# wangtong627/COR

Measured on AMD Instinct MI355X. Metric: query triplets/sec (forward + similarity + top-k), higher is better.
Workload: dtype bf16

## Files before the change

cor_amd/_native.py:

```python
from __future__ import annotations

import ctypes as C
import os

_HERE = os.path.dirname(os.path.abspath(__file__))
LIB_PATH = os.environ.get("COR_AMD_LIB") or os.path.join(_HERE, "csrc", "libcor_amd.so")

F32, BF16, F16, BF16X3 = 0, 1, 2, 3
ACT_NONE, ACT_GELU_ERF, ACT_RELU, ACT_SIGMOID, ACT_GELU_TANH = 0, 1, 2, 3, 4
EINVAL, ENOSUPPORT = -1, -2
TOPK_FORCE_LISTS, TOPK_NO_FALLBACK, TOPK_FORCE_GLOBAL_THRESHOLD, TOPK_WAVE_FINAL = 1, 2, 8, 16
TOPK_KMAX = 256
FILTER_EQ, FILTER_NE = 0, 1
MERGE_NMAX = 4096
EXPAND_SEGMAX = 16
ORDER_REVERSE = 1 << 30
KERNEL_ROWLANE, KERNEL_FEWQ, KERNEL_FLASH_MFMA, KERNEL_FLASH_PIPELINED, KERNEL_WINDOW_BLOCK = 1, 2, 3, 4, 5
import numpy as _np
Q_PRESCALE_HD64 = float(_np.float32(0.125) * _np.float32(1.4426950408889634))

_p, _i, _l, _f, _ll = C.c_void_p, C.c_int, C.c_long, C.c_float, C.c_longlong

SIGNATURES = {
    "cor_version": [],
    "cor_gemm": [_p, _l, _p, _l, _i, _p, _l, _i, _i, _i, _i, _p, _i, _p, _p, _l, _i, _i, _p],
    "cor_layernorm": [_p, _i, _p, _i, _p, _p, _i, _i, _f, _i, _p],
    "cor_attention": [_p, _l, _l, _p, _l, _l, _p, _l, _l, _i, _p, _l, _l, _i, _i, _i, _i, _i, _i, _f, _p],
    "cor_attention_f32": [_p, _l, _l, _p, _l, _l, _p, _l, _l, _p, _l, _l, _i, _i, _i, _i, _i, _i, _f, _p],
    "cor_attention_kernel_id": [_i, _i, _i, _i, _i, _i],
    "cor_sam_attention": [_p, _i, _p, _i, _p, _p, _p, _i, _i, _i, _i, _i, _f, _i, _p],
    "cor_patchify": [_p, _p, _i, _i, _i, _i, _i, _i, _i, _p],
    "cor_im2col3x3": [_p, _i, _p, _i, _i, _i, _i, _p],
    "cor_add": [_p, _i, _p, _i, _p, _i, _l, _l, _p],
    "cor_copy_rows": [_p, _l, _i, _p, _l, _i, _i, _i, _p],
    "cor_split_x3": [_p, _l, _p, _l, _l, _i, _i, _p],
    "cor_tokens_to_nchw": [_p, _i, _p, _i, _i, _i, _p],
    "cor_nchw_to_tokens": [_p, _p, _i, _i, _i, _i, _p],
    "cor_l2norm_rows": [_p, _i, _p, _i, _i, _i, _f, _p],
    "cor_embed_tokens": [_p, _p, _p, _p, _i, _i, _i, _i, _p],
    "cor_bilinear": [_p, _p, _i, _i, _i, _i, _i, _i, _p],
    "cor_conv3x3s2_small": [_p, _i, _p, _p, _p, _i, _i, _i, _i, _i, _p],
    "cor_dwconv7x7": [_p, _p, _p, _p, _i, _i, _i, _i, _i, _p],
    "cor_adapter_pool": [_p, _p, _p, _i, _i, _i, _i, _p],
    "cor_masked_pool": [_p, _i, _p, _p, _i, _i, _i, _i, _i, _p],
    "cor_region_pool": [_p, _p, _p, _p, _i, _i, _i, _i, _i, _i, _i, _p],
    "cor_fuse_gate": [_p, _p, _p, _p, _p, _i, _i, _p],
    "cor_fuse_mix": [_p, _p, _p, _i, _i, _p],
    "cor_dense_pe": [_p, _p, _i, _i, _p],
    "cor_upscale_shuffle": [_p, _i, _p, _p, _p, _f, _i, _p, _i, _i, _i, _i, _i, _p],
    "cor_upscale_hyper": [_p, _i, _p, _p, _p, _l, _p, _i, _i, _i, _i, _i, _i, _p],
    "cor_iou_select": [_p, _p, _i, _i, _i, _i, _i, _p, _p, _p],
    "cor_decoder_heads": [_p, _p, _p, _p, _p, _i, _p, _p, _i, _p],
    "cor_mask_prob_minmax": [_p, _p, _i, _i, _p],
    "cor_resize_binarize": [_p, _p, _i, _i, _i, _i, _i, _f, _p],
    "cor_resize_gray": [_p, _p, _i, _i, _i, _i, _i, _p],
# ... 60 lines not shown
```

cor_amd/csrc/flash_attn.hip:

```cpp
#include <cstdlib>
#include <type_traits>

#include "common.h"

typedef short s16x4 __attribute__((ext_vector_type(4)));

namespace {

struct FlashArgs {
  const bf16_t* q; const bf16_t* k; const bf16_t* v; void* o;
  long q_sb, q_st, k_sb, k_st, v_sb, v_st, o_sb, o_st;
  int H, Tq, Tk;
  float scale_log2;
  float tbl_scale;
  const bf16_t* pad_row; const float* rel_h; const float* rel_w;
  int grid, S, nW, d3;
  int nqt;
  int rev;
};

constexpr int KT = 64;
constexpr int TILE_B = KT * 128;
constexpr int KV_BYTES = 4 * TILE_B;
constexpr int AUX_PER_WAVE = 8192;
// ... 1034 lines not shown
    const unsigned lds0 = __builtin_amdgcn_readfirstlane((unsigned)(size_t)((__attribute__((address_space(3))) char*)smem));
    const int sl = lane & 7;
    long colp[2]; bool okx[2];
#pragma unroll
    for (int hf = 0; hf < 2; ++hf) {
      const int kw = min(8 * hf + (lane >> 3), 13), x = wx * 14 + kw;
      okx[hf] = x < a.grid;
      colp[hf] = ((long)b * g2 + x) * a.d3 + head * 64;
    }
#pragma unroll
    for (int i8 = 0; i8 < 8; ++i8) {
      const int i = wave * 8 + i8;
      const bool isv = i >= 28;
      const int ii = isv ? i - 28 : i, kh = ii >> 1, hf = ii & 1, y = wy * 14 + kh;
      const int chunk = isv ? (sl ^ (((lane >> 4) & 1) << 2)) : (sl ^ (4 * hf + (lane >> 4)));
      const long plane = (long)(isv ? 2 : 1) * a.H * 64 + chunk * 8;
      const bf16_t* src = (y < a.grid && okx[hf]) ? a.q + colp[hf] + (long)y * a.grid * a.d3 + plane : a.pad_row + head * 64 + plane;
      glds16(src, lds0 + (isv ? WIN_KV : 0) + ii * 1024);
    }
  }

  const int tq = min(wave * 32 + r, 195);
  const int qh = (tq * 4682) >> 16, qw = tq - 14 * qh;
  uint4 qf[4];
  {
    const int y = wy * 14 + qh, x = wx * 14 + qw;
    const bf16_t* qp = (y < a.grid && x < a.grid) ? a.q + ((long)b * g2 + (long)y * a.grid + x) * a.d3 + head * 64 : a.pad_row + head * 64;
#pragma unroll
    for (int c = 0; c < 4; ++c) qf[c] = *(const uint4*)(qp + 16 * c + 8 * h);
  }

  float colb[8];
  uint4 tf[2][4];
#pragma unroll
  for (int tbl = 0; tbl < 2; ++tbl)
#pragma unroll
    for (int c = 0; c < 4; ++c) tf[tbl][c] = table_frag(tbl == 0 ? a.rel_w : a.rel_h, min(r, 26), c, h);
#pragma unroll
  for (int tbl = 0; tbl < 2; ++tbl) {
    f32x16 acc;
#pragma unroll
    for (int e = 0; e < 16; ++e) acc[e] = 0.f;
#pragma unroll
    for (int c = 0; c < 4; ++c)
      acc = __builtin_amdgcn_mfma_f32_32x32x16_bf16(__builtin_bit_cast(bf16x8, tf[tbl][c]), __builtin_bit_cast(bf16x8, qf[c]), acc, 0, 0, 0);
#pragma unroll
    for (int e = 0; e < 16; ++e) {
      const int row = acc_row(e, h);
      if (row < 27) T[row * 32 + r] = acc[e] * a.tbl_scale;
    }
    __builtin_amdgcn_fence(__ATOMIC_ACQ_REL, "wavefront");
    if (tbl == 0) {
#pragma unroll
      for (int e8 = 0; e8 < 8; ++e8) {
        const int kw = (e8 & 3) + 8 * (e8 >> 2) + 4 * h;
        colb[e8] = kw < 14 ? T[(qw - min(kw, 13) + 13) * 32 + r] : -INFINITY;
      }
      __builtin_amdgcn_fence(__ATOMIC_ACQ_REL, "wavefront");
    }
  }

  if (a.scale_log2 != 1.0f) {
#pragma unroll
    for (int c = 0; c < 4; ++c) {
      uint32_t w[4] = {qf[c].x, qf[c].y, qf[c].z, qf[c].w};
#pragma unroll
      for (int i = 0; i < 4; ++i) w[i] = pk2(__uint_as_float(w[i] << 16) * a.scale_log2, __uint_as_float(w[i] & 0xffff0000u) * a.scale_log2);
      qf[c] = make_uint4(w[0], w[1], w[2], w[3]);
    }
  }

  asm volatile("s_waitcnt vmcnt(0)" ::: "memory");
  __syncthreads();

  const int sw = (r >> 1) & 7;
  const int k_rd = r * 128, v_tr = (4 * h + ((lane & 15) >> 2)) * 128 + (16 * ((lane >> 4) & 1) + 4 * (lane & 3)) * 2;
  const int v_trd[2] = {v_tr + ((lane >> 3) & 1) * 64, v_tr + (1 - ((lane >> 3) & 1)) * 64};
  const int t_rd = (qh + 13) * 32 + r;
  f32x16 o[2], lsum;
#pragma unroll
  for (int e = 0; e < 16; ++e) { o[0][e] = 0.f; o[1][e] = 0.f; lsum[e] = 0.f; }
  float m = 0.f;
  const uint4 ones = make_uint4(0x3F803F80u, 0x3F803F80u, 0x3F803F80u, 0x3F803F80u);
#pragma unroll
  for (int blk = 0; blk < 7; ++blk) {
    const char* Kb = Kt + blk * 32 * 128 + k_rd;
    uint4 kf[4];
#pragma unroll
    for (int c = 0; c < 4; ++c) kf[c] = *(const uint4*)(Kb + (((2 * c + h) ^ sw) << 4));
    const float rm0 = T[t_rd - 32 * (2 * blk)] - m, rm1 = T[t_rd - 32 * (2 * blk + 1)] - m;
    f32x16 s;
#pragma unroll
    for (int e = 0; e < 16; ++e) s[e] = colb[e & 7] + (e < 8 ? rm0 : rm1);
#pragma unroll
    for (int c = 0; c < 4; ++c)
      s = __builtin_amdgcn_mfma_f32_32x32x16_bf16(__builtin_bit_cast(bf16x8, kf[c]), __builtin_bit_cast(bf16x8, qf[c]), s, 0, 0, 0);
// ... 234 lines not shown
```

cor_amd/csrc/gemm.hip:

```cpp
#include "common.h"

#ifdef COR_PROBES
#define COR_DBG(g_, bit_) ((g_).dbg & (bit_))
#else
#define COR_DBG(g_, bit_) 0
#endif
#ifndef COR_GEMM_DEFAULT_BIG
#define COR_GEMM_DEFAULT_BIG 2
#endif

namespace {

struct GemmArgs {
  const char* A; const char* W; char* C;
  long lda_b, ldw_b;
  long ldc;
  int M, N, Kb;
  int tm, tn;
  const float* bias; const float* col_scale; const float* residual;
  long ldr; int res_row_mod; int act;
  int group_m;
  unsigned long long* stamps;
  int dbg;
  int vec_epi;
  int rev;
  int nt_c;
  int order;
};

template <typename TA> struct Mfma;
template <> struct Mfma<float> {
  static __device__ __forceinline__ void run(const uint4& a, const uint4& b, f32x16& acc) {
    acc = __builtin_amdgcn_mfma_f32_32x32x2f32(__uint_as_float(a.x), __uint_as_float(b.x), acc, 0, 0, 0);
    acc = __builtin_amdgcn_mfma_f32_32x32x2f32(__uint_as_float(a.y), __uint_as_float(b.y), acc, 0, 0, 0);
    acc = __builtin_amdgcn_mfma_f32_32x32x2f32(__uint_as_float(a.z), __uint_as_float(b.z), acc, 0, 0, 0);
    acc = __builtin_amdgcn_mfma_f32_32x32x2f32(__uint_as_float(a.w), __uint_as_float(b.w), acc, 0, 0, 0);
  }
};
template <> struct Mfma<bf16_t> {
  static __device__ __forceinline__ void run(const uint4& a, const uint4& b, f32x16& acc) {
    acc = __builtin_amdgcn_mfma_f32_32x32x16_bf16(__builtin_bit_cast(bf16x8, a), __builtin_bit_cast(bf16x8, b), acc, 0, 0, 0);
  }
};

__device__ __forceinline__ void mfma16_bf16(const uint4& a, const uint4& b, f32x4& acc) {
  acc = __builtin_amdgcn_mfma_f32_16x16x32_bf16(__builtin_bit_cast(bf16x8, a), __builtin_bit_cast(bf16x8, b), acc, 0, 0, 0);
}

constexpr int ROWB = 128;

template <int ACT, typename TO = float> __device__ __forceinline__ float act_ct(float v) {
// ... 68 lines not shown
          st4<TO>(cp, v[0]);
        }
      }
    }
  }
}

template <typename TO, int MI, int NJ, int WTN>
__device__ __forceinline__ void epilogue_vec(const f32x16 (&acc)[MI][NJ], float* stg, const GemmArgs& g, int mbase, int nbase,
                                             int lane) {
#define COR_EPI(A_)                                                                                            \
  if (g.residual) epilogue_vec_ct<TO, MI, NJ, WTN, A_, true>(acc, stg, g, mbase, nbase, lane);                \
  else epilogue_vec_ct<TO, MI, NJ, WTN, A_, false>(acc, stg, g, mbase, nbase, lane);
  switch (g.act) {
    case COR_ACT_GELU_ERF: COR_EPI(COR_ACT_GELU_ERF) break;
    case COR_ACT_RELU: COR_EPI(COR_ACT_RELU) break;
    case COR_ACT_SIGMOID: COR_EPI(COR_ACT_SIGMOID) break;
    case COR_ACT_GELU_TANH: COR_EPI(COR_ACT_GELU_TANH) break;
    default: COR_EPI(COR_ACT_NONE) break;
  }
#undef COR_EPI
}

template <typename TA, typename TO, int BM, int BN, int WM, int WN, bool GLDS, int NBUF = 2>
__global__ void __launch_bounds__(WM * WN * 64, ((BM / WM) * (BN / WN) >= 8192 && WM * WN == 4) ? 1 : 2)
gemm_tile(const GemmArgs g) {
  constexpr int NT = WM * WN * 64;
  constexpr int WTM = BM / WM, WTN = BN / WN, MI = WTM / 32, NJ = WTN / 32;
  constexpr int A_BYTES = BM * ROWB, B_BYTES = BN * ROWB, BUF = A_BYTES + B_BYTES;
  constexpr int ACH = BM * 8 / NT, BCH = BN * 8 / NT;
  extern __shared__ __attribute__((aligned(16))) char smem[];
  const int tid = threadIdx.x, lane = tid & 63, wave = tid >> 6;
  const int wm = wave / WN, wn = wave % WN;
  const int swz0 = xcd_remap(blockIdx.x, gridDim.x);
  const int swz = g.rev ? (int)gridDim.x - 1 - swz0 : swz0;
  const int GM = g.group_m;
  const int band = swz / (GM * g.tn), rem = swz - band * (GM * g.tn);
  const int gm_eff = min(GM, g.tm - band * GM);
  const int m0 = (band * GM + rem % gm_eff) * BM, n0 = (rem / gm_eff) * BN;

  const char* a_src[ACH]; const char* b_src[BCH]; int a_ko[ACH], b_ko[BCH];
#pragma unroll
  for (int i = 0; i < ACH; ++i) {
    const int c = tid + NT * i, row = c >> 3, ch = (c & 7) ^ ((row >> 1) & 7);
    a_src[i] = g.A + (long)min(m0 + row, g.M - 1) * g.lda_b + ch * 16;
    a_ko[i] = ch * 16;
  }
#pragma unroll
  for (int i = 0; i < BCH; ++i) {
    const int c = tid + NT * i, row = c >> 3, ch = (c & 7) ^ ((row >> 1) & 7);
    b_src[i] = g.W + (long)min(n0 + row, g.N - 1) * g.ldw_b + ch * 16;
    b_ko[i] = ch * 16;
  }
  const unsigned wslot = __builtin_amdgcn_readfirstlane(tid & ~63) * 16;
  const unsigned lds0 = __builtin_amdgcn_readfirstlane((unsigned)(size_t)((__attribute__((address_space(3))) char*)smem));

  const int r = lane & 31, h = lane >> 5, sw = (lane >> 1) & 7;
  const int a_rd = (wm * WTM + r) * ROWB, b_rd = A_BYTES + (wn * WTN + r) * ROWB;
  int ch_rd[4];
#pragma unroll
  for (int s = 0; s < 4; ++s) ch_rd[s] = ((2 * s + h) ^ sw) << 4;

  f32x16 acc[MI][NJ];
#pragma unroll
  for (int i = 0; i < MI; ++i)
#pragma unroll
    for (int j = 0; j < NJ; ++j)
#pragma unroll
      for (int e = 0; e < 16; ++e) acc[i][j][e] = 0.0f;

  const int nkt = (g.Kb + ROWB - 1) / ROWB;
  uint4 ra[GLDS ? 1 : ACH], rb[GLDS ? 1 : BCH];

  auto stage_issue = [&](int kt, int buf) {
    const int kb = kt * ROWB;
    if constexpr (GLDS) {
      const unsigned base = lds0 + buf * BUF + wslot;
#pragma unroll
      for (int i = 0; i < ACH; ++i) glds16(a_src[i] + kb, base + NT * 16 * i);
#pragma unroll
      for (int i = 0; i < BCH; ++i) glds16(b_src[i] + kb, base + A_BYTES + NT * 16 * i);
    } else {
#pragma unroll
      for (int i = 0; i < ACH; ++i)
        ra[i] = (kb + a_ko[i] + 16 <= g.Kb) ? *(const uint4*)(a_src[i] + kb) : make_uint4(0, 0, 0, 0);
#pragma unroll
      for (int i = 0; i < BCH; ++i)
        rb[i] = (kb + b_ko[i] + 16 <= g.Kb) ? *(const uint4*)(b_src[i] + kb) : make_uint4(0, 0, 0, 0);
    }
  };
  auto stage_commit = [&](int buf) {
    if constexpr (!GLDS) {
      char* base = smem + buf * BUF + tid * 16;
#pragma unroll
      for (int i = 0; i < ACH; ++i) *(uint4*)(base + NT * 16 * i) = ra[i];
#pragma unroll
      for (int i = 0; i < BCH; ++i) *(uint4*)(base + A_BYTES + NT * 16 * i) = rb[i];
    }
  };
// ... 204 lines not shown
    __builtin_amdgcn_fence(__ATOMIC_ACQUIRE, "wavefront");
#pragma unroll
    for (int p4 = 0; p4 < 4; ++p4) {
      const int row = p4 * 8 + rr0;
      const uint4 q = *(const uint4*)(stg + row * 128 + ((cvr ^ ((row >> 1) & 7)) << 4));
      const int m = mbase + mi * 32 + row, n = nbase + cvr * 8;
      const unsigned off = (m < g.M && n < g.N) ? (unsigned)(((long)m * g.ldc + n) * 2L) : 0xFFFFFFFFu;
      u32x4 u; u[0] = q.x; u[1] = q.y; u[2] = q.z; u[3] = q.w;
      if constexpr (NT) __builtin_amdgcn_raw_buffer_store_b128(u, crs, off, 0, 2);
      else if (COR_DBG(g, 0x2000)) __builtin_amdgcn_raw_buffer_store_b128(u, crs, off, 0, 2);
      else if (COR_DBG(g, 0x4000)) __builtin_amdgcn_raw_buffer_store_b128(u, crs, off, 0, 16);
      else __builtin_amdgcn_raw_buffer_store_b128(u, crs, off, 0, 0);
    }
    __builtin_amdgcn_fence(__ATOMIC_RELEASE, "wavefront");
    __builtin_amdgcn_fence(__ATOMIC_ACQUIRE, "wavefront");
  }
}

#define COR_VMCNT(n_) asm volatile("s_waitcnt vmcnt(" #n_ ")" ::: "memory")

#define COR_BAR() asm volatile("s_barrier" ::: "memory")
#define COR_LGKM0() asm volatile("s_waitcnt lgkmcnt(0)" ::: "memory")

template <typename TO, bool M16>
__global__ void __launch_bounds__(512, 1) gemm_pp(const GemmArgs g) {
  constexpr int BM = 256, BN = 256, HT = 16384, NSLOT = 10;
  constexpr int MI = 4, NJ = 2, WTM = 128, WTN = 64;
  constexpr int VW = sizeof(TO) == 2 ? 8 : 4;
  constexpr int NSTORE = MI * NJ * (32 / (64 / (32 / VW)));
  static_assert(NSTORE == 16 || NSTORE == 32, "counted waits below");
  constexpr bool CT = sizeof(TO) == 2 && !M16;
  extern __shared__ __attribute__((aligned(16))) char smem[];
  const int tid = threadIdx.x, lane = tid & 63, wave = tid >> 6;
  const int wr = wave >> 2, wc = wave & 3;
  const unsigned lds0 = __builtin_amdgcn_readfirstlane((unsigned)(size_t)((__attribute__((address_space(3))) char*)smem));
  const unsigned wslot = __builtin_amdgcn_readfirstlane(wave) * 1024u;

  const int srow = tid >> 3, sch = ((tid & 7) ^ ((tid >> 4) & 7)) * 16;
  const int r = M16 ? (lane & 15) : (lane & 31), h = lane >> 5, q = lane >> 4, sw = (r >> 1) & 7;
  int chs[4];
#pragma unroll
  for (int s4 = 0; s4 < 4; ++s4) chs[s4] = M16 ? (((4 * (s4 & 1) + q) ^ sw) << 4) : (((2 * s4 + h) ^ sw) << 4);
  const int a_row = r * 128;
  const int b_row = ((wc & 1) * 64 + r) * 128;

  const int nkt = g.Kb / 128;
  const int total = g.tm * g.tn, G = gridDim.x;
  const int GM = g.group_m;
  const __amdgpu_buffer_rsrc_t crs = __builtin_amdgcn_make_buffer_rsrc(
      g.C, 0, (int)(unsigned)((((long)g.M - 1) * g.ldc + g.N) * (long)sizeof(TO)), 0x00020000);

  unsigned oa[4], ob[4];
  int m0 = 0, n0 = 0;
  const int per_xcd = (total + 7) >> 3;
// ... 180 lines not shown
      }
    };
    float* stg = (float*)(smem + 4 * HT) + wave * 1024;
    const int mb = cm0 + wr * WTM, nb = cn0 + wc * WTN;
    auto bias_col = [&](int nj, int jb) -> int { return M16 ? nj * 32 + jb * 16 + r : nj * 32 + r; };
    auto fill = [&](int mi, int nj, float* st, const float (&b)[2]) {
      if constexpr (M16) {
#pragma unroll
        for (int ib = 0; ib < 2; ++ib)
#pragma unroll
          for (int jb = 0; jb < 2; ++jb)
#pragma unroll
            for (int e = 0; e < 4; ++e) st[(ib * 16 + q * 4 + e) * 32 + jb * 16 + r] = acc16[2 * mi + ib][2 * nj + jb][e] + b[jb];
      } else {
#pragma unroll
        for (int e = 0; e < 16; ++e) st[((e & 3) + 8 * (e >> 2) + 4 * h) * 32 + r] = acc[mi][nj][e] + b[0];
      }
    };
    auto accv = [&](int mi, int nj, int e) -> float { if constexpr (M16) return 0.0f; else return acc[mi][nj][e]; };
#define COR_EPI(A_)                                                                                             \
    if constexpr (CT) {                                                                                         \
      if (g.nt_c) epilogue_ct16<MI, NJ, A_, true>(accv, pre, (char*)stg, g, crs, mb, nb, lane);                \
      else epilogue_ct16<MI, NJ, A_, false>(accv, pre, (char*)stg, g, crs, mb, nb, lane);                      \
    } else                                                                                                      \
    if (g.residual) epilogue_buf_ct<TO, MI, NJ, A_, true, false>(fill, pre, bias_col, stg, g, crs, mb, nb, lane, qi - 1);  \
    else if (sizeof(TO) == 2 && g.nt_c) epilogue_buf_ct<TO, MI, NJ, A_, false, sizeof(TO) == 2>(fill, pre, bias_col, stg, g, crs, mb, nb, lane); \
    else epilogue_buf_ct<TO, MI, NJ, A_, false, false>(fill, pre, bias_col, stg, g, crs, mb, nb, lane);
    if (COR_DBG(g, 2)) {
      pre();
      float t = 0.f;
      if constexpr (M16) {
#pragma unroll
        for (int i = 0; i < 8; ++i)
#pragma unroll
          for (int j = 0; j < 4; ++j) t += acc16[i][j][0] + acc16[i][j][3];
      } else {
#pragma unroll
        for (int i = 0; i < MI; ++i)
#pragma unroll
          for (int j = 0; j < NJ; ++j) t += acc[i][j][0] + acc[i][j][15];
      }
      if (t == 1.2345f) ((float*)g.C)[tid] = t;
    } else
    switch (g.act) {
      case COR_ACT_GELU_ERF: COR_EPI(COR_ACT_GELU_ERF) break;
      case COR_ACT_RELU: COR_EPI(COR_ACT_RELU) break;
// ... 30 lines not shown
    __syncthreads();
#pragma unroll 8
    for (int kk = 0; kk < 32; ++kk) {
      const float w = Ws[tx][kk];
#pragma unroll
      for (int i = 0; i < 4; ++i) acc[i] = fmaf(As[ty + 8 * i][kk], w, acc[i]);
    }
    __syncthreads();
  }
  const int n = n0 + tx;
  if (n >= N) return;
  const float bv = bias ? bias[n] : 0.0f, sc = col_scale ? col_scale[n] : 1.0f;
#pragma unroll
  for (int i = 0; i < 4; ++i) {
    const int m = m0 + ty + 8 * i;
    if (m >= M) continue;
    float v = (sizeof(TO) == 2 && act == COR_ACT_GELU_ERF ? gelu_erf_bf16out_f(acc[i] + bv) : apply_act(acc[i] + bv, act)) * sc;
    if (residual) v += residual[(long)(res_row_mod > 0 ? m % res_row_mod : m) * ldr + n];
    st<TO>(C + (long)m * ldc + n, v);
  }
}


template <typename TA, typename TO, int BM, int BN, int WM, int WN, bool GLDS, int NBUF = 2>
int launch_tile(GemmArgs g, hipStream_t s) {
  constexpr int LDS = NBUF * (BM + BN) * ROWB;
  g.tm = cdiv(g.M, BM); g.tn = cdiv(g.N, BN);
  static DevOnce once;
  cor_max_dyn_lds((const void*)gemm_tile<TA, TO, BM, BN, WM, WN, GLDS, NBUF>, LDS, once);
  hipLaunchKernelGGL((gemm_tile<TA, TO, BM, BN, WM, WN, GLDS, NBUF>), dim3(g.tm * g.tn), dim3(WM * WN * 64), LDS, s, g);
  COR_CHECK_LAUNCH();
  return 0;
}

template <typename TA, typename TO>
int launch_gemm(const void* A, long lda, const void* W, long ldw, void* C, long ldc, int M, int N, int K,
                const float* bias, int act, const float* col_scale, const float* residual, long ldr, int res_row_mod,
                int cfg_arg, hipStream_t s) {
  const int g_gemm_cfg = cfg_arg & 0xff, g_gemm_dbg = (cfg_arg & ~COR_ORDER_REVERSE) >> 8;
  const long esz = sizeof(TA);
  const bool fast = (K * esz) % 16 == 0 && (lda * esz) % 16 == 0 && (ldw * esz) % 16 == 0 &&
                    ((uintptr_t)A % 16 == 0) && ((uintptr_t)W % 16 == 0);
  if (!fast) {
    hipLaunchKernelGGL((gemm_nt_small<TA, TO>), dim3(cdiv(N, 32), cdiv(M, 32)), dim3(256), 0, s, (const TA*)A, lda,
                       (const TA*)W, ldw, (TO*)C, ldc, M, N, K, bias, act, col_scale, residual, ldr, res_row_mod);
    COR_CHECK_LAUNCH();
    return 0;
  }
  GemmArgs g;
  g.A = (const char*)A; g.W = (const char*)W; g.C = (char*)C;
  g.lda_b = lda * esz; g.ldw_b = ldw * esz; g.ldc = ldc;
  g.M = M; g.N = N; g.Kb = (int)(K * esz);
  g.stamps = nullptr;
#ifdef COR_PROBES
  if (g_gemm_dbg & 0x100000) { g.stamps = (unsigned long long*)col_scale; col_scale = nullptr; }
#endif
  g.bias = bias; g.col_scale = col_scale; g.residual = residual; g.ldr = ldr; g.res_row_mod = res_row_mod; g.act = act;
  g.dbg = g_gemm_dbg & 0x3fefff; g.rev = (cfg_arg & COR_ORDER_REVERSE) ? 1 : 0;
  g.order = 1;
  g.nt_c = (sizeof(TO) == 2 && !residual) ? 1 : 0;
  g.group_m = ((g_gemm_dbg >> 4) & 0xff) ? ((g_gemm_dbg >> 4) & 0xff) : 8;
  const auto al16 = [](const void* p) { return ((uintptr_t)p & 15) == 0; };
  g.vec_epi = (N % 4 == 0) && (N >= 8) && (ldc % (sizeof(TO) == 2 ? 8 : 4) == 0) && al16(C) && (!bias || al16(bias)) && (!col_scale || al16(col_scale)) &&
              (!residual || (al16(residual) && ldr % 4 == 0));
  const bool k128 = g.Kb % ROWB == 0;
  int cfg = g_gemm_cfg;
  if (cfg == 0) {
    cfg = (k128 && M >= 512 && N >= 64) ? ((N <= 256 && K >= 2048 && M >= 65536) ? 9 : COR_GEMM_DEFAULT_BIG) : 1;
    if (k128 && M < 512 && N >= 64) cfg = 4;
    if (cfg == 2 && (long)cdiv(M, 128) * cdiv(N, 128) < 256) cfg = 4;
    else if (cfg == 2 && (long)cdiv(M, 128) * cdiv(N, 128) < 512) cfg = 3;
    if (sizeof(TA) == 2 && k128 && !col_scale && (long)cdiv(M, 256) * cdiv(N, 256) >= 140 && 4L * N >= 3L * 256 * cdiv(N, 256) && K >= 256) cfg = 13;
  }
  if (!k128 && (cfg == 2 || cfg == 3 || cfg == 4)) cfg = 1;
  if (cfg == 13 || cfg == 14) {
    const long c_bytes = (((long)M - 1) * ldc + N) * (long)sizeof(TO);
    const bool ok = sizeof(TA) == 2 && k128 && g.vec_epi && !col_scale && N % 8 == 0 && c_bytes < (1L << 32) - 64 && !(sizeof(TO) == 2 && residual) &&
                    (long)M * g.lda_b < (1L << 32) && (long)N * g.ldw_b < (1L << 32);
    if (!ok) cfg = k128 ? 2 : 1;
    else if constexpr (sizeof(TA) == 2) {
      g.tm = cdiv(g.M, 256); g.tn = cdiv(g.N, 256);
      g.order = g.tn <= 4 ? 1 : 0;
      if (g_gemm_dbg & 0x1000) g.order ^= 1;
      static DevOnce once_a;
      const int n_cu = cor_device_cus();
      cor_max_dyn_lds((const void*)gemm_pp<TO, false>, 163840, once_a);
#ifdef COR_PROBES
      static DevOnce once_b;
      cor_max_dyn_lds((const void*)gemm_pp<TO, true>, 163840, once_b);
#endif
      const int total = g.tm * g.tn;
      int blocks = n_cu - (n_cu & 7);
      if (total < blocks) blocks = ((total + 7) / 8) * 8;
#ifdef COR_PROBES
      if (cfg == 14) hipLaunchKernelGGL((gemm_pp<TO, true>), dim3(blocks), dim3(512), 163840, s, g);
      else
#endif
      hipLaunchKernelGGL((gemm_pp<TO, false>), dim3(blocks), dim3(512), 163840, s, g);
      COR_CHECK_LAUNCH();
      return 0;
    }
  }
  if (!k128 && cfg >= 9) cfg = 1;
  switch (cfg) {
    case 9: return launch_tile<TA, TO, 256, 128, 4, 2, true, 3>(g, s);
    case 2: return launch_tile<TA, TO, 128, 128, 2, 2, true>(g, s);
    case 3: return launch_tile<TA, TO, 128, 64, 2, 2, true>(g, s);
    case 4: return launch_tile<TA, TO, 64, 64, 2, 2, true>(g, s);
    default: return launch_tile<TA, TO, 128, 128, 2, 2, false>(g, s);
  }
}

}

extern "C" int cor_gemm(const void* A, long lda, const void* W, long ldw, int ab_dtype, void* C, long ldc, int c_dtype,
                        int M, int N, int K, const float* bias, int act, const float* col_scale,
                        const float* residual, long ldr, int res_row_mod, int cfg, void* stream) {
  if (!A || !W || !C || M <= 0 || N <= 0 || K <= 0 || lda < K || ldw < K || ldc < N) return COR_EINVAL;
  {
    const int sel = cfg & 0xff;
#ifdef COR_PROBES
    if (cfg < 0 || sel > 14) return COR_EINVAL;
#else
    if (cfg < 0 || (cfg & ~(0xff | COR_ORDER_REVERSE)) != 0 || !(sel == 0 || sel == 1 || sel == 2 || sel == 3 || sel == 4 || sel == 9 || sel == 13)) return COR_EINVAL;
#endif
  }
  if (residual && ldr < N) return COR_EINVAL;
  if (ab_dtype == COR_BF16X3) {
    if (lda < 3L * K || ldw < 3L * K || K > (1 << 29)) return COR_EINVAL;
    ab_dtype = COR_BF16;
    K *= 3;
  }
  hipStream_t s = (hipStream_t)stream;
  if (ab_dtype == COR_F32 && c_dtype == COR_F32)
    return launch_gemm<float, float>(A, lda, W, ldw, C, ldc, M, N, K, bias, act, col_scale, residual, ldr, res_row_mod, cfg, s);
// ... 9 lines not shown
```

cor_amd/engine.py:

```python
from __future__ import annotations

import math

import torch

from . import _native as nat
from . import ops
from .ops import ACT_NONE, ACT_GELU_ERF, ACT_RELU, ACT_SIGMOID, ACT_GELU_TANH, X3

F32 = torch.float32


def _round_up(x, m):
    return (x + m - 1) // m * m


class _Packer:

    def __init__(self, sd: dict, T: torch.dtype):
        dev = next(iter(sd.values())).device
        if dev.type != "cuda":
            raise RuntimeError("cor_amd: the model must live on a GPU (model.to('cuda')); there is no CPU path")
        self.sd, self.T, self.W = sd, T, {}

# ... 160 lines not shown
def _gelu(kind):
    return ACT_GELU_ERF if kind == "erf" else ACT_GELU_TANH


def sam_encoder(W, img, cfg, T, p="image_encoder."):
    B = img.shape[0]
    g, d, H = cfg["img"] // cfg["patch"], cfg["dim"], cfg["heads"]
    assert img.shape[1:] == (3, cfg["img"], cfg["img"]), f"SAM input must be [B,3,{cfg['img']},{cfg['img']}], got {tuple(img.shape)}"
    cols = ops.patchify(img, cfg["patch"], W[p + "patch.K"], T)
    x = ops.gemm(cols, W[p + "patch_embed.proj.weight"], out_dtype=F32, bias=W[p + "patch_embed.proj.bias"],
                 residual=W[p + "pos_embed"], res_row_mod=g * g)
    del cols
    for i in range(cfg["depth"]):
        b = f"{p}blocks.{i}."
        win = 0 if i in cfg["global_idx"] else cfg["window"]
        h = _ln(W, b + "norm1.", x, 1e-6, T, reverse=True)
        qkv = _lin(W, b + "attn.qkv.", h, T)
        a = ops.sam_attention(qkv, W[b + "attn.pad_row"], W[b + "attn.rel_pos_h"], W[b + "attn.rel_pos_w"], B, H, g, win,
                              q_prescale=W[b + "attn.q_prescale"], reverse=True)
        del qkv
        _lin(W, b + "attn.proj.", a, F32, residual=x, out=x)
        h = _ln(W, b + "norm2.", x, 1e-6, T, reverse=True)
        m = _lin(W, b + "mlp.lin1.", h, T, act=ACT_GELU_ERF)
        _lin(W, b + "mlp.lin2.", m, F32, residual=x, out=x)
        del h, a, m
    y = ops.gemm(ops.cast(x, T), W[p + "neck.0.weight"], out_dtype=F32)
    y = _ln(W, p + "neck.1.", y, 1e-6, T)
    y = ops.gemm(ops.im2col3x3(y, B, g, g), W[p + "neck.2.weight"], out_dtype=F32)
    return _ln(W, p + "neck.3.", y, 1e-6, F32)


def _vit_mha(qkv, N, Tn, heads, D, T):
    hd = D // heads
    if T == X3:
        return ops.attention_f32(qkv[:, 0:D], qkv[:, D:2 * D], qkv[:, 2 * D:3 * D], N, heads, Tn, Tn, hd, hd ** -0.5, out_dtype=X3)
    return ops.attention(qkv[:, 0:D], qkv[:, D:2 * D], qkv[:, 2 * D:3 * D], N, heads, Tn, Tn, hd, hd ** -0.5, out_dtype=T)


def _qkv_dtype(T):
    return F32 if T == X3 else T


def siglip_vision(W, img, g, T, p="support_branch.siglip.model.visual.trunk."):
    N = img.shape[0]
    D, P = g["dim"], (g["image"] // g["patch"]) ** 2
    x3 = T == X3
    assert img.shape[1:] == (3, g["image"], g["image"]), f"SigLIP input must be [N,3,{g['image']},{g['image']}], got {tuple(img.shape)}"
    cols = ops.patchify(img, g["patch"], W[p + "patch.K"], T)
    x = ops.gemm(cols, W[p + "patch_embed.proj.weight"], out_dtype=F32, bias=W[p + "patch_embed.proj.bias"],
                 residual=W[p + "pos_embed"], res_row_mod=P, x3=x3)
    act = _gelu(g.get("v_gelu", g.get("gelu", "erf")))
# ... 249 lines not shown
```

cor_amd/ops.py:

```python
from __future__ import annotations

import torch

from . import _native as nat
from ._native import ACT_NONE, ACT_GELU_ERF, ACT_RELU, ACT_SIGMOID, ACT_GELU_TANH, F32, BF16, F16

_DT = {torch.float32: F32, torch.bfloat16: BF16, torch.float16: F16}

X3 = "bf16x3"

GEMM_PROFILE = None


def _lib():
    return nat.load()


def _dt(t: torch.Tensor) -> int:
    return _DT[t.dtype]


def _s():
    return torch.cuda.current_stream().cuda_stream

# ... 137 lines not shown
    out = torch.empty((B * grid * grid, d), dtype=out_dtype or qkv.dtype, device=qkv.device)
    nat.check(_lib().cor_sam_attention(qkv.data_ptr(), _dt(qkv), out.data_ptr(), _dt(out), _p(pad_row), rel_h.data_ptr(),
                                       rel_w.data_ptr(), B, H, hd, grid, window, float(q_prescale), int(variant) | (nat.ORDER_REVERSE if reverse else 0), _s()), "cor_sam_attention")
    return out


def patchify(img, p, Kpad, out_dtype):
    if out_dtype == X3:
        return split_x3(patchify(img, p, Kpad, torch.float32))
    _dev(img)
    assert img.dtype == torch.float32 and img.is_contiguous() and img.dim() == 4
    B, C, H, W = img.shape
    out = torch.empty((B * (H // p) * (W // p), Kpad), dtype=out_dtype, device=img.device)
    nat.check(_lib().cor_patchify(img.data_ptr(), out.data_ptr(), _dt(out), B, C, H, W, p, Kpad, _s()), "cor_patchify")
    return out


def im2col3x3(x, B, H, W):
    _dev(x)
    C = x.shape[-1]
    assert x.is_contiguous() and x.numel() == B * H * W * C
    out = torch.empty((B * H * W, 9 * C), dtype=x.dtype, device=x.device)
    nat.check(_lib().cor_im2col3x3(x.data_ptr(), _dt(x), out.data_ptr(), B, H, W, C, _s()), "cor_im2col3x3")
    return out


def add(a, b, out_dtype=None, out=None):
    _dev(a, b, out)
    assert a.is_contiguous() and b.is_contiguous() and a.numel() % b.numel() == 0
    if out is None:
        out = torch.empty(a.shape, dtype=out_dtype or a.dtype, device=a.device)
    assert out.is_contiguous() and out.numel() == a.numel()
    nat.check(_lib().cor_add(a.data_ptr(), _dt(a), b.data_ptr(), _dt(b), out.data_ptr(), _dt(out), a.numel(), b.numel(), _s()),
              "cor_add")
    return out


def copy_rows(src_ptr_tensor, ld_in, rows, C, out, ld_out=None, src_offset=0):
    _dev(src_ptr_tensor, out)
    src = src_ptr_tensor
    assert src.is_contiguous()
    need = src_offset + (rows - 1) * ld_in + C
    assert need <= src.numel(), (need, src.numel())
    if ld_out is None:
        ld_out = out.stride(0) if out.dim() == 2 else C
    assert out.stride(-1) == 1
# ... 440 lines not shown
```

include/cor_amd.h:

```cpp
#ifndef COR_AMD_H
#define COR_AMD_H

#ifdef __cplusplus
extern "C" {
#endif

#define COR_EINVAL (-1)
#define COR_ENOSUPPORT (-2)
#define COR_ORDER_REVERSE (1 << 30)
#define COR_TOPK_FORCE_LISTS 1
#define COR_TOPK_NO_FALLBACK 2
#define COR_TOPK_FORCE_GLOBAL_THRESHOLD 8
#define COR_TOPK_WAVE_FINAL 16
#define COR_TOPK_KMAX 256
#define COR_MERGE_NMAX 4096
#define COR_FILTER_EQ 0
#define COR_FILTER_NE 1

enum { COR_F32 = 0, COR_BF16 = 1, COR_F16 = 2 , COR_BF16X3 = 3  };
enum { COR_ACT_NONE = 0, COR_ACT_GELU_ERF = 1, COR_ACT_RELU = 2, COR_ACT_SIGMOID = 3, COR_ACT_GELU_TANH = 4 };

int cor_version(void);


// ... 6 lines not shown
                  int rows, int C, float eps, int act, void* stream);


int cor_attention(const void* q, long q_sb, long q_st, const void* k, long k_sb, long k_st,
                  const void* v, long v_sb, long v_st, int dtype,
                  void* out, long o_sb, long o_st, int out_dtype,
                  int B, int H, int Tq, int Tk, int hd, float scale, void* stream);

int cor_attention_f32(const float* q, long q_sb, long q_st, const float* k, long k_sb, long k_st,
                      const float* v, long v_sb, long v_st, void* out, long o_sb, long o_st, int out_dtype,
                      int B, int H, int Tq, int Tk, int hd, float scale, void* stream);

int cor_sam_attention(const void* qkv, int dtype, void* out, int out_dtype, const void* pad_row,
                      const float* rel_h, const float* rel_w, int B, int H, int hd, int grid, int window, float q_prescale, int variant,
                      void* stream);

enum { COR_KERNEL_ROWLANE = 1, COR_KERNEL_FEWQ = 2, COR_KERNEL_FLASH_MFMA = 3, COR_KERNEL_FLASH_PIPELINED = 4, COR_KERNEL_WINDOW_BLOCK = 5 };
int cor_attention_kernel_id(int dtype, int hd, int Tq, int Tk, int sam_window, int grid);


int cor_patchify(const float* img, void* out, int out_dtype, int B, int C, int H, int W, int p, int Kpad, void* stream);

int cor_im2col3x3(const void* x, int dtype, void* out, int B, int H, int W, int C, void* stream);

int cor_add(const void* a, int a_dtype, const void* b, int b_dtype, void* out, int out_dtype, long n, long b_period, void* stream);

int cor_copy_rows(const void* in, long ld_in, int in_dtype, void* out, long ld_out, int out_dtype, int rows, int C, void* stream);

int cor_split_x3(const float* in, long ld_in, void* out, long ld_out, long seg, int rows, int C, void* stream);

int cor_tokens_to_nchw(const void* x, int dtype, float* out, int B, int HW, int C, void* stream);
int cor_nchw_to_tokens(const float* x, void* out, int out_dtype, int B, int HW, int C, void* stream);

int cor_l2norm_rows(const void* x, int x_dtype, void* y, int y_dtype, int rows, int C, float eps, void* stream);

int cor_embed_tokens(const long long* ids, const float* table, const float* pos, float* out, int rows, int ctx, int D, int vocab, void* stream);


int cor_bilinear(const float* x, float* out, int planes, int H, int W, int OH, int OW, int clamp01, void* stream);

int cor_conv3x3s2_small(const float* x, int x_channels_last, const float* w, const float* bias, float* out,
                        int B, int Cin, int Cout, int H, int W, void* stream);

int cor_dwconv7x7(const float* x, const float* w_t, const float* bias, void* out, int out_dtype, int B, int H, int W, int C, void* stream);

int cor_adapter_pool(const float* maps, const float* feat, float* out, int B, int P, int M, int D, void* stream);
// ... 75 lines not shown
```

Before: 777.8.

## Add implicit 3x3 conv GEMM, bf16 residual epilogue, and skip dead attention waves

Adds an implicit-convolution mode to the tiled GEMM that gathers the 3x3 neighbourhood taps straight from token rows via LDS-DMA, with a zero line for padding. The neck conv uses it instead of materialising a 9x im2col buffer and then running a separate GEMM. It also adds a bf16-output residual epilogue for the persistent GEMM, so the last block's MLP projection can write bf16 directly. Separately, windowed attention waves whose query rows all fall into padding now skip their loads and compute. The trade-offs are added kernel complexity, an extra template instantiation, and a possible small precision change from storing the last residual in bf16.

Result: no change. 783.8, median of 6 (+0.8%).

```diff
diff --git a/cor_amd/_native.py b/cor_amd/_native.py
--- a/cor_amd/_native.py
+++ b/cor_amd/_native.py
@@ -31,6 +31,7 @@
     "cor_sam_attention": [_p, _i, _p, _i, _p, _p, _p, _i, _i, _i, _i, _i, _f, _i, _p],
     "cor_patchify": [_p, _p, _i, _i, _i, _i, _i, _i, _i, _p],
     "cor_im2col3x3": [_p, _i, _p, _i, _i, _i, _i, _p],
+    "cor_conv3x3_tokens": [_p, _p, _l, _p, _l, _i, _i, _i, _i, _i, _i, _p],
     "cor_add": [_p, _i, _p, _i, _p, _i, _l, _l, _p],
     "cor_copy_rows": [_p, _l, _i, _p, _l, _i, _i, _i, _p],
     "cor_split_x3": [_p, _l, _p, _l, _l, _i, _i, _p],
diff --git a/cor_amd/csrc/flash_attn.hip b/cor_amd/csrc/flash_attn.hip
--- a/cor_amd/csrc/flash_attn.hip
+++ b/cor_amd/csrc/flash_attn.hip
@@ -1080,7 +1080,10 @@
 
   const int tq = min(wave * 32 + r, 195);
   const int qh = (tq * 4682) >> 16, qw = tq - 14 * qh;
+  const bool live = __builtin_amdgcn_ballot_w64(wave * 32 + r < 196 && wy * 14 + qh < a.grid && wx * 14 + qw < a.grid) != 0;
   uint4 qf[4];
+  float colb[8];
+  if (live) {
   {
     const int y = wy * 14 + qh, x = wx * 14 + qw;
     const bf16_t* qp = (y < a.grid && x < a.grid) ? a.q + ((long)b * g2 + (long)y * a.grid + x) * a.d3 + head * 64 : a.pad_row + head * 64;
@@ -1088,7 +1091,6 @@
     for (int c = 0; c < 4; ++c) qf[c] = *(const uint4*)(qp + 16 * c + 8 * h);
   }
 
-  float colb[8];
   uint4 tf[2][4];
 #pragma unroll
   for (int tbl = 0; tbl < 2; ++tbl)
@@ -1128,8 +1130,11 @@
     }
   }
 
+  }
+
   asm volatile("s_waitcnt vmcnt(0)" ::: "memory");
   __syncthreads();
+  if (!live) return;
 
   const int sw = (r >> 1) & 7;
   const int k_rd = r * 128, v_tr = (4 * h + ((lane & 15) >> 2)) * 128 + (16 * ((lane >> 4) & 1) + 4 * (lane & 3)) * 2;
diff --git a/cor_amd/csrc/gemm.hip b/cor_amd/csrc/gemm.hip
--- a/cor_amd/csrc/gemm.hip
+++ b/cor_amd/csrc/gemm.hip
@@ -26,7 +26,10 @@
   int rev;
   int nt_c;
   int order;
+  int conv_h, conv_w;
 };
+
+__device__ __attribute__((aligned(128))) unsigned int g_conv_zero_line[32];
 
 template <typename TA> struct Mfma;
 template <> struct Mfma<float> {
@@ -141,9 +144,10 @@
 #undef COR_EPI
 }
 
-template <typename TA, typename TO, int BM, int BN, int WM, int WN, bool GLDS, int NBUF = 2>
+template <typename TA, typename TO, int BM, int BN, int WM, int WN, bool GLDS, int NBUF = 2, bool CONV = false>
 __global__ void __launch_bounds__(WM * WN * 64, ((BM / WM) * (BN / WN) >= 8192 && WM * WN == 4) ? 1 : 2)
 gemm_tile(const GemmArgs g) {
+  static_assert(!CONV || (GLDS && NBUF == 3), "implicit convolution: LDS-DMA staging, three buffers");
   constexpr int NT = WM * WN * 64;
   constexpr int WTM = BM / WM, WTN = BN / WN, MI = WTM / 32, NJ = WTN / 32;
   constexpr int A_BYTES = BM * ROWB, B_BYTES = BN * ROWB, BUF = A_BYTES + B_BYTES;
@@ -159,11 +163,22 @@
   const int m0 = (band * GM + rem % gm_eff) * BM, n0 = (rem / gm_eff) * BN;
 
   const char* a_src[ACH]; const char* b_src[BCH]; int a_ko[ACH], b_ko[BCH];
+  unsigned a_taps[CONV ? ACH : 1];
 #pragma unroll
   for (int i = 0; i < ACH; ++i) {
     const int c = tid + NT * i, row = c >> 3, ch = (c & 7) ^ ((row >> 1) & 7);
-    a_src[i] = g.A + (long)min(m0 + row, g.M - 1) * g.lda_b + ch * 16;
+    const int m = min(m0 + row, g.M - 1);
+    a_src[i] = g.A + (long)m * g.lda_b + ch * 16;
     a_ko[i] = ch * 16;
+    if constexpr (CONV) {
+      const int pix = m % (g.conv_h * g.conv_w), y = pix / g.conv_w, x = pix - y * g.conv_w;
+      const unsigned rowm = (y > 0 ? 1u : 0u) | 2u | (y + 1 < g.conv_h ? 4u : 0u);
+      const unsigned colm = (x > 0 ? 1u : 0u) | 2u | (x + 1 < g.conv_w ? 4u : 0u);
+      unsigned t9 = 0;
+#pragma unroll
+      for (int t = 0; t < 9; ++t) t9 |= (((rowm >> (t / 3)) & (colm >> (t % 3))) & 1u) << t;
+      a_taps[i] = t9;
+    }
   }
 #pragma unroll
   for (int i = 0; i < BCH; ++i) {
@@ -191,9 +206,21 @@
   const int nkt = (g.Kb + ROWB - 1) / ROWB;
   uint4 ra[GLDS ? 1 : ACH], rb[GLDS ? 1 : BCH];
 
+  int cv_tap = 0, cv_ofs = 0;
   auto stage_issue = [&](int kt, int buf) {
     const int kb = kt * ROWB;
-    if constexpr (GLDS) {
+    if constexpr (CONV) {
+      const unsigned base = lds0 + buf * BUF + wslot;
+      const int dy = cv_tap / 3 - 1, dx = cv_tap - 3 * (dy + 1) - 1;
+      const long shift = (long)(dy * g.conv_w + dx) * g.lda_b + cv_ofs;
+      const char* zl = (const char*)g_conv_zero_line;
+#pragma unroll
+      for (int i = 0; i < ACH; ++i) glds16(((a_taps[i] >> cv_tap) & 1u) ? a_src[i] + shift : zl + a_ko[i], base + NT * 16 * i);
+#pragma unroll
+      for (int i = 0; i < BCH; ++i) glds16(b_src[i] + kb, base + A_BYTES + NT * 16 * i);
+      cv_ofs += ROWB;
+      if (cv_ofs >= (int)g.lda_b) { cv_ofs = 0; ++cv_tap; }
+    } else if constexpr (GLDS) {
       const unsigned base = lds0 + buf * BUF + wslot;
 #pragma unroll
       for (int i = 0; i < ACH; ++i) glds16(a_src[i] + kb, base + NT * 16 * i);
@@ -444,14 +471,15 @@
 #define COR_BAR() asm volatile("s_barrier" ::: "memory")
 #define COR_LGKM0() asm volatile("s_waitcnt lgkmcnt(0)" ::: "memory")
 
-template <typename TO, bool M16>
+template <typename TO, bool M16, bool RB = false>
 __global__ void __launch_bounds__(512, 1) gemm_pp(const GemmArgs g) {
   constexpr int BM = 256, BN = 256, HT = 16384, NSLOT = 10;
   constexpr int MI = 4, NJ = 2, WTM = 128, WTN = 64;
   constexpr int VW = sizeof(TO) == 2 ? 8 : 4;
   constexpr int NSTORE = MI * NJ * (32 / (64 / (32 / VW)));
   static_assert(NSTORE == 16 || NSTORE == 32, "counted waits below");
-  constexpr bool CT = sizeof(TO) == 2 && !M16;
+  static_assert(!RB || (sizeof(TO) == 2 && !M16), "RB: bf16 C + fp32 residual, 32x32 MFMAs");
+  constexpr bool CT = sizeof(TO) == 2 && !M16 && !RB;
   extern __shared__ __attribute__((aligned(16))) char smem[];
   const int tid = threadIdx.x, lane = tid & 63, wave = tid >> 6;
   const int wr = wave >> 2, wc = wave & 3;
@@ -678,6 +706,8 @@
     if constexpr (CT) {                                                                                         \
       if (g.nt_c) epilogue_ct16<MI, NJ, A_, true>(accv, pre, (char*)stg, g, crs, mb, nb, lane);                \
       else epilogue_ct16<MI, NJ, A_, false>(accv, pre, (char*)stg, g, crs, mb, nb, lane);                      \
+    } else if constexpr (RB) {                                                                                  \
+      epilogue_buf_ct<TO, MI, NJ, A_, true, false>(fill, pre, bias_col, stg, g, crs, mb, nb, lane, qi - 1);     \
     } else                                                                                                      \
     if (g.residual) epilogue_buf_ct<TO, MI, NJ, A_, true, false>(fill, pre, bias_col, stg, g, crs, mb, nb, lane, qi - 1);  \
     else if (sizeof(TO) == 2 && g.nt_c) epilogue_buf_ct<TO, MI, NJ, A_, false, sizeof(TO) == 2>(fill, pre, bias_col, stg, g, crs, mb, nb, lane); \
@@ -754,13 +784,13 @@
 }
 
 
-template <typename TA, typename TO, int BM, int BN, int WM, int WN, bool GLDS, int NBUF = 2>
+template <typename TA, typename TO, int BM, int BN, int WM, int WN, bool GLDS, int NBUF = 2, bool CONV = false>
 int launch_tile(GemmArgs g, hipStream_t s) {
   constexpr int LDS = NBUF * (BM + BN) * ROWB;
   g.tm = cdiv(g.M, BM); g.tn = cdiv(g.N, BN);
   static DevOnce once;
-  cor_max_dyn_lds((const void*)gemm_tile<TA, TO, BM, BN, WM, WN, GLDS, NBUF>, LDS, once);
-  hipLaunchKernelGGL((gemm_tile<TA, TO, BM, BN, WM, WN, GLDS, NBUF>), dim3(g.tm * g.tn), dim3(WM * WN * 64), LDS, s, g);
+  cor_max_dyn_lds((const void*)gemm_tile<TA, TO, BM, BN, WM, WN, GLDS, NBUF, CONV>, LDS, once);
+  hipLaunchKernelGGL((gemm_tile<TA, TO, BM, BN, WM, WN, GLDS, NBUF, CONV>), dim3(g.tm * g.tn), dim3(WM * WN * 64), LDS, s, g);
   COR_CHECK_LAUNCH();
   return 0;
 }
@@ -790,6 +820,7 @@
   g.bias = bias; g.col_scale = col_scale; g.residual = residual; g.ldr = ldr; g.res_row_mod = res_row_mod; g.act = act;
   g.dbg = g_gemm_dbg & 0x3fefff; g.rev = (cfg_arg & COR_ORDER_REVERSE) ? 1 : 0;
   g.order = 1;
+  g.conv_h = g.conv_w = 0;
   g.nt_c = (sizeof(TO) == 2 && !residual) ? 1 : 0;
   g.group_m = ((g_gemm_dbg >> 4) & 0xff) ? ((g_gemm_dbg >> 4) & 0xff) : 8;
   const auto al16 = [](const void* p) { return ((uintptr_t)p & 15) == 0; };
@@ -807,7 +838,7 @@
   if (!k128 && (cfg == 2 || cfg == 3 || cfg == 4)) cfg = 1;
   if (cfg == 13 || cfg == 14) {
     const long c_bytes = (((long)M - 1) * ldc + N) * (long)sizeof(TO);
-    const bool ok = sizeof(TA) == 2 && k128 && g.vec_epi && !col_scale && N % 8 == 0 && c_bytes < (1L << 32) - 64 && !(sizeof(TO) == 2 && residual) &&
+    const bool ok = sizeof(TA) == 2 && k128 && g.vec_epi && !col_scale && N % 8 == 0 && c_bytes < (1L << 32) - 64 &&
                     (long)M * g.lda_b < (1L << 32) && (long)N * g.ldw_b < (1L << 32);
     if (!ok) cfg = k128 ? 2 : 1;
     else if constexpr (sizeof(TA) == 2) {
@@ -824,11 +855,19 @@
       const int total = g.tm * g.tn;
       int blocks = n_cu - (n_cu & 7);
       if (total < blocks) blocks = ((total + 7) / 8) * 8;
+      bool launched = false;
 #ifdef COR_PROBES
-      if (cfg == 14) hipLaunchKernelGGL((gemm_pp<TO, true>), dim3(blocks), dim3(512), 163840, s, g);
-      else
+      if (cfg == 14) { hipLaunchKernelGGL((gemm_pp<TO, true>), dim3(blocks), dim3(512), 163840, s, g); launched = true; }
 #endif
-      hipLaunchKernelGGL((gemm_pp<TO, false>), dim3(blocks), dim3(512), 163840, s, g);
+      if constexpr (sizeof(TO) == 2) {
+        if (!launched && residual) {
+          static DevOnce once_r;
+          cor_max_dyn_lds((const void*)gemm_pp<TO, false, true>, 163840, once_r);
+          hipLaunchKernelGGL((gemm_pp<TO, false, true>), dim3(blocks), dim3(512), 163840, s, g);
+          launched = true;
+        }
+      }
+      if (!launched) hipLaunchKernelGGL((gemm_pp<TO, false>), dim3(blocks), dim3(512), 163840, s, g);
       COR_CHECK_LAUNCH();
       return 0;
     }
@@ -843,6 +882,25 @@
   }
 }
 
+}
+
+extern "C" int cor_conv3x3_tokens(const void* x, const void* w, long ldw, float* out, long ldc, int B, int H, int W, int C, int N,
+                                  int cfg, void* stream) {
+  if (!x || !w || !out || B <= 0 || H <= 0 || W <= 0 || C <= 0 || N <= 0) return COR_EINVAL;
+  if ((C * 2L) % ROWB != 0) return COR_EINVAL;
+  if (cfg != 0 && cfg != COR_ORDER_REVERSE) return COR_EINVAL;
+  const long M = (long)B * H * W, K = 9L * C;
+  if (ldw < K || ldc < N || M >= (1L << 31) || K * 2 >= (1L << 31) || (((uintptr_t)x | (uintptr_t)w) & 15) != 0 || (ldw * 2) % 16 != 0) return COR_EINVAL;
+  GemmArgs g;
+  g.A = (const char*)x; g.W = (const char*)w; g.C = (char*)out;
+  g.lda_b = C * 2L; g.ldw_b = ldw * 2; g.ldc = ldc;
+  g.M = (int)M; g.N = N; g.Kb = (int)(K * 2);
+  g.stamps = nullptr;
+  g.bias = nullptr; g.col_scale = nullptr; g.residual = nullptr; g.ldr = 0; g.res_row_mod = 0; g.act = COR_ACT_NONE;
+  g.dbg = 0; g.rev = (cfg & COR_ORDER_REVERSE) ? 1 : 0; g.order = 1; g.nt_c = 0; g.group_m = 8;
+  g.vec_epi = (N % 4 == 0) && (N >= 8) && (ldc % 4 == 0) && (((uintptr_t)out & 15) == 0);
+  g.conv_h = H; g.conv_w = W;
+  return launch_tile<bf16_t, float, 256, 128, 4, 2, true, 3, true>(g, (hipStream_t)stream);
 }
 
 extern "C" int cor_gemm(const void* A, long lda, const void* W, long ldw, int ab_dtype, void* C, long ldc, int c_dtype,
diff --git a/cor_amd/engine.py b/cor_amd/engine.py
--- a/cor_amd/engine.py
+++ b/cor_amd/engine.py
@@ -206,11 +206,18 @@
         _lin(W, b + "attn.proj.", a, F32, residual=x, out=x)
         h = _ln(W, b + "norm2.", x, 1e-6, T, reverse=True)
         m = _lin(W, b + "mlp.lin1.", h, T, act=ACT_GELU_ERF)
-        _lin(W, b + "mlp.lin2.", m, F32, residual=x, out=x)
+        if i == cfg["depth"] - 1 and T == torch.bfloat16:
+            x = _lin(W, b + "mlp.lin2.", m, T, residual=x)
+        else:
+            _lin(W, b + "mlp.lin2.", m, F32, residual=x, out=x)
         del h, a, m
     y = ops.gemm(ops.cast(x, T), W[p + "neck.0.weight"], out_dtype=F32)
     y = _ln(W, p + "neck.1.", y, 1e-6, T)
-    y = ops.gemm(ops.im2col3x3(y, B, g, g), W[p + "neck.2.weight"], out_dtype=F32)
+    w3 = W[p + "neck.2.weight"]
+    if ops.conv3x3_tokens_supported(y, B, g, g, w3.shape[0]):
+        y = ops.conv3x3_tokens(y, w3, B, g, g)
+    else:
+        y = ops.gemm(ops.im2col3x3(y, B, g, g), w3, out_dtype=F32)
     return _ln(W, p + "neck.3.", y, 1e-6, F32)
 
 
diff --git a/cor_amd/ops.py b/cor_amd/ops.py
--- a/cor_amd/ops.py
+++ b/cor_amd/ops.py
@@ -183,6 +183,31 @@
     assert x.is_contiguous() and x.numel() == B * H * W * C
     out = torch.empty((B * H * W, 9 * C), dtype=x.dtype, device=x.device)
     nat.check(_lib().cor_im2col3x3(x.data_ptr(), _dt(x), out.data_ptr(), B, H, W, C, _s()), "cor_im2col3x3")
+    return out
+
+
+def conv3x3_tokens_supported(x, B, H, W, N):
+    C = x.shape[-1]
+    return x.dtype == torch.bfloat16 and (C * 2) % 128 == 0 and 9 * C >= 2048 and B * H * W >= 65536 and 64 <= N <= 256
+
+
+def conv3x3_tokens(x, w, B, H, W, reverse=False):
+    _dev(x, w)
+    C = x.shape[-1]
+    assert x.dtype == torch.bfloat16 and w.dtype == torch.bfloat16 and x.is_contiguous() and x.numel() == B * H * W * C
+    N, K, ldw = _rows(w)
+    assert K == 9 * C, (w.shape, C)
+    out = torch.empty((B * H * W, N), dtype=torch.float32, device=x.device)
+    prof = GEMM_PROFILE
+    if prof is not None:
+        e0, e1 = torch.cuda.Event(enable_timing=True), torch.cuda.Event(enable_timing=True)
+        e0.record()
+    nat.check(_lib().cor_conv3x3_tokens(x.data_ptr(), w.data_ptr(), ldw, out.data_ptr(), N, B, H, W, C, N,
+                                        nat.ORDER_REVERSE if reverse else 0, _s()), "cor_conv3x3_tokens")
+    if prof is not None:
+        e1.record()
+        M = B * H * W
+        prof.append((e0, e1, 2.0 * M * N * K, x.dtype, float((M * C + N * K) * 2 + M * N * 4)))
     return out
 
 
diff --git a/include/cor_amd.h b/include/cor_amd.h
--- a/include/cor_amd.h
+++ b/include/cor_amd.h
@@ -52,6 +52,9 @@
 int cor_patchify(const float* img, void* out, int out_dtype, int B, int C, int H, int W, int p, int Kpad, void* stream);
 
 int cor_im2col3x3(const void* x, int dtype, void* out, int B, int H, int W, int C, void* stream);
+
+int cor_conv3x3_tokens(const void* x, const void* w, long ldw, float* out, long ldc, int B, int H, int W, int C, int N, int cfg,
+                       void* stream);
 
 int cor_add(const void* a, int a_dtype, const void* b, int b_dtype, void* out, int out_dtype, long n, long b_period, void* stream);
 
```
